# joshspeagle/dynesty

Measured on AMD Instinct MI355X. Metric: proposals/sec + ellipsoid-rebuilds/sec, 25-D corr-Normal nlive=2000 (multi/rwalk), higher is better.
Workload: dtype f64; 1 GPU; C2 x 64 independent runs per GPU (C5 shard); per step and run: 1 MultiEllipsoid rebuild + enlarge 1.25 + 4 queue fills of K=512 walkers x 45 rwalk steps (= one bound-update interval at the queue size that passes the ln Z gate); live sets uniform inside the likelihood contour; ndim=25, nlive=2000, walks=45, queue_size=512, runs_per_gpu=64, tap_point=A (kernel boundary), rebuild_in_step=True, rng=PCG64 + ziggurat, stream-identical to numpy.random.Generator (parity mode)

## Files before the change

### dynesty_amd/csrc/rebuild.hip

```cpp
#include <math.h>
#include <stdlib.h>

#include "ctx.h"
#include <type_traits>
#include <vector>
#include "eig_wave.h"

using namespace dh;
using dh_eig::jacobi_wave;
using dh_eig::sort_eigs_wave;
using dh_eig::wave_sync;

namespace {

constexpr int kThreads = 256;
constexpr double kRoundDelta = 1e-3;
constexpr double kMaxCond = 1e12;
constexpr double kEigMult = 10.0;
constexpr int kNTries = 100;

struct Node {
  int start, count;
  int parent, child0, child1;
  int depth;
// ... 1202 lines not shown
    PH_ADD(15);
    return L.lam[0] > 0.0 && isfinite(L.lam[0]);
  }
  __shared__ double s_q;
  if (t < 64) {
    double y = 0.0;
    if (t < D)
      for (int k = 0; k < D; ++k) y = fma(L.AX[t * LD + k], s_v[k], y);
    const double q = wave_sum(t < D ? y * s_v[t] : 0.0);
    if (t == 0) s_q = q;
  }
  __syncthreads();
  {
    const double q = s_q, rq = sqrt(q);
    for (int e = t; e < D * D; e += NT) {
      const int i = e / D, jj = e - i * D, o = i * LD + jj;
      Q[o] = L.AX[o];
      L.AX[o] = jj == 0 ? s_v[i] * rq : 0.0;
    }
    if (t < D) L.lam[t] = t == 0 ? q : 0.0;
    if (cov_keep) *cov_keep = Q;
    __syncthreads();
    PH_ADD(15);
    return q > 0.0 && isfinite(q);
  }
}

template <int NT = kThreads>
__device__ __forceinline__ int ellipsoid_finish_fast(const Lds& L, const RebuildArgs& a, double* es, double* cov_g,
                                                     const double* cov_keep, double fmx, double logdet,
                                                     double* logvol_out) {
  const int D = a.d, t = threadIdx.x, LD = L.LD, DD = D * D;
  if (!isfinite(logdet)) return DH_ERR_VALUE;
  const double lim = 1.0 - kRoundDelta;
  const bool sc = fmx > lim;
  const double mult = fmx / lim, rt = sqrt(mult);
  if (t < D) {
    st_c(L, es + t, L.mean[t]);
    double lam = L.lam[t];
    if (sc) lam *= mult;
    st_c(L, es + D + 3 * DD + t, sqrt(lam));
  }
  for (int e = t; e < DD; e += NT) {
    const int i = e / D, j = e - i * D, o = i * LD + j;
    double c = cov_keep[o], am = L.AM[o], ax = L.AX[o];
    if (sc) {
      c *= mult;
      am /= mult;
      ax *= rt;
      cov_g[o] = c;
    }
    st_c(L, es + D + e, c);
    st_c(L, es + D + DD + e, am);
    st_c(L, es + D + 2 * DD + e, ax);
  }
  *logvol_out = a.prefactor + 0.5 * logdet;
  return DH_OK;
}

template <int NT = kThreads>
__device__ __forceinline__ void ellipsoid_rescale(const Lds& L, double* cov_g, int D, double fmx) {
  const int t = threadIdx.x, LD = L.LD;
  const double lim = 1.0 - kRoundDelta;
  if (fmx > lim) {
    const double mult = fmx / lim;
    const double rt = sqrt(mult);
    for (int e = t; e < D * D; e += NT) {
      const int i = e / D, j = e % D;
      cov_g[i * LD + j] *= mult;
      L.AM[i * LD + j] /= mult;
      L.AX[i * LD + j] *= rt;
    }
    __syncthreads();
    if (t < D) L.lam[t] *= mult;
    __syncthreads();
  }
}

__device__ __forceinline__ int ellipsoid_store(const Lds& L, const RebuildArgs& a, double* es, const double* cov_g,
                                               double* logvol_out) {
  const int D = a.d, t = threadIdx.x, LD = L.LD;
  bool ok = true;
  double slog = 0.0;
  for (int k = 0; k < D; ++k) {
    const double l = L.lam[k];
    if (!(l > 0.0) || !isfinite(l)) ok = false;
    slog += log(l);
  }
  if (!ok) return DH_ERR_VALUE;
  const double logvol = a.prefactor + 0.5 * slog;
  const int DD = D * D;
  if (t < D) {
    st_c(L, es + t, L.mean[t]);
    st_c(L, es + D + 3 * DD + t, sqrt(L.lam[t]));
  }
  for (int e = t; e < DD; e += kThreads) {
    const int i = e / D, j = e % D;
    st_c(L, es + D + e, cov_g[i * LD + j]);
    st_c(L, es + D + DD + e, L.AM[i * LD + j]);
    st_c(L, es + D + 2 * DD + e, L.AX[i * LD + j]);
  }
  __syncthreads();
  *logvol_out = logvol;
  return DH_OK;
}

template <int NT = kThreads>
__device__ __forceinline__ int ellipsoid_store_fast(const Lds& L, const RebuildArgs& a, double* es,
                                                    const double* cov_g, double logdet, double* logvol_out) {
  const int D = a.d, t = threadIdx.x, LD = L.LD;
  if (!isfinite(logdet)) return DH_ERR_VALUE;
  const int DD = D * D;
  if (t < D) {
    st_c(L, es + t, L.mean[t]);
    st_c(L, es + D + 3 * DD + t, sqrt(L.lam[t]));
  }
  for (int e = t; e < DD; e += NT) {
    const int i = e / D, j = e % D;
    st_c(L, es + D + e, cov_g[i * LD + j]);
    st_c(L, es + D + DD + e, L.AM[i * LD + j]);
    st_c(L, es + D + 2 * DD + e, L.AX[i * LD + j]);
  }
  __syncthreads();
  *logvol_out = a.prefactor + 0.5 * logdet;
  return DH_OK;
}

constexpr int kFullRecord = 1;

constexpr int kDeferred = 3;
template <bool FAST, bool CHILD = false>
__device__ __forceinline__ int node_ellipsoid(const Lds& L, const RebuildArgs& a, const double* pts, const int* perm,
                                              int start, int count, double* es, double* cov_g, double* logvol_out,
                                              double* fmax_out, bool have_mean = false) {
  const int D = a.d, t = threadIdx.x, LD = L.LD;
  if (count == 1) return DH_ERR_VALUE;
  PH_T0();
  if (CHILD || have_mean) {
    if (t < D) L.mean[t] = ld_c(L, es + t);
    __syncthreads();
  } else {
    node_mean(L, pts, perm, start, count, D);
  }
  PH_ADD(0);
  int fused = 0;
  node_cov(L, pts, perm, start, count, D, CHILD ? false : !have_mean, FAST ? cov_g : nullptr, &fused);
  PH_ADD(1);
  if (!fused) {
    for (int e = t; e < D * D; e += kThreads) cov_g[(e / D) * LD + e % D] = L.A[(e / D) * LD + e % D];
    __syncthreads();
  }
  if constexpr (FAST) {
    double logdet = 0.0;
    const double* cov_keep = nullptr;
    if (fused != 2 && spd_fast(L, cov_g, D, a.mode == 0 && count >= 4 * D, &logdet, &cov_keep, fused == 1)) {
      const double fmx = node_fmax(L, pts, perm, start, count, D);
      PH_ADD(3);
      if (fmx > 1.0 - kRoundDelta) logdet += (double)D * log(fmx / (1.0 - kRoundDelta));
      *fmax_out = fmin(fmx, 1.0 - kRoundDelta);
      if (cov_keep != nullptr) return ellipsoid_finish_fast(L, a, es, cov_g, cov_keep, fmx, logdet, logvol_out);
      ellipsoid_rescale(L, cov_g, D, fmx);
      return ellipsoid_store_fast(L, a, es, cov_g, logdet, logvol_out);
    }
    if constexpr (CHILD) return kDeferred;
    __syncthreads();
    for (int pass = 0; pass < 2; ++pass) {
      const bool good = regularize<false>(L, cov_g, D);
      const double fmx = node_fmax(L, pts, perm, start, count, D);
      if (pass == 0) ellipsoid_rescale(L, cov_g, D, fmx);
      if (pass == 1 && fmx >= 1.0) return DH_ERR_CONTAIN;
      *fmax_out = pass == 0 ? fmin(fmx, 1.0 - kRoundDelta) : fmx;
      if (good) break;
    }
    const int rc = ellipsoid_store(L, a, es, cov_g, logvol_out);
    return rc == DH_OK ? kFullRecord : rc;
  } else {
    for (int pass = 0; pass < 2; ++pass) {
      const bool good = regularize(L, cov_g, D);
      PH_ADD(2);
      const double fmx = node_fmax(L, pts, perm, start, count, D);
      PH_ADD(3);
      if (pass == 0) ellipsoid_rescale(L, cov_g, D, fmx);
      if (pass == 1 && fmx >= 1.0) return DH_ERR_CONTAIN;
      *fmax_out = pass == 0 ? fmin(fmx, 1.0 - kRoundDelta) : fmx;
      if (good) break;
    }
    return ellipsoid_store(L, a, es, cov_g, logvol_out);
  }
}


constexpr int kBarSleep = 4;
__device__ __forceinline__ void drain_stores() {
  __builtin_amdgcn_s_waitcnt(0x0F70);
}

typedef double dh_d2 __attribute__((ext_vector_type(2)));
__device__ __forceinline__ void st_agent16(double* p, double v, unsigned long long tag) {
  dh_d2 x;
  x.x = v;
  x.y = __longlong_as_double((long long)tag);
  asm volatile("global_store_dwordx4 %0, %1, off sc1\n\ts_nop 1" ::"v"(p), "v"(x) : "memory");
}
__device__ __forceinline__ void ld_agent16x8(const double* const (&p)[8], dh_d2 (&v)[8]) {
  asm volatile(
      "global_load_dwordx4 %0, %8, off sc1\n\t"
      "global_load_dwordx4 %1, %9, off sc1\n\t"
      "global_load_dwordx4 %2, %10, off sc1\n\t"
      "global_load_dwordx4 %3, %11, off sc1\n\t"
      "global_load_dwordx4 %4, %12, off sc1\n\t"
      "global_load_dwordx4 %5, %13, off sc1\n\t"
      "global_load_dwordx4 %6, %14, off sc1\n\t"
      "global_load_dwordx4 %7, %15, off sc1\n\t"
      "s_waitcnt vmcnt(0)"
      : "=&v"(v[0]), "=&v"(v[1]), "=&v"(v[2]), "=&v"(v[3]), "=&v"(v[4]), "=&v"(v[5]), "=&v"(v[6]), "=&v"(v[7])
      : "v"(p[0]), "v"(p[1]), "v"(p[2]), "v"(p[3]), "v"(p[4]), "v"(p[5]), "v"(p[6]), "v"(p[7])
      : "memory");
}

template <bool MAXOP = false>
__device__ __forceinline__ double tagged_partner_reduce(const double* base, size_t stride, int col, int np,
                                                        unsigned long long tag, bool* ok) {
  double acc = MAXOP ? -INFINITY : 0.0;
  for (int pp0 = 0; pp0 < np && *ok; pp0 += 8) {
    const double* ptr[8];
    dh_d2 v[8];
#pragma unroll
    for (int uu = 0; uu < 8; ++uu) ptr[uu] = base + ((size_t)min(pp0 + uu, np - 1) * stride + col) * 2;
    for (int spins = 0;; ++spins) {
      ld_agent16x8(ptr, v);
      bool all = true;
#pragma unroll
      for (int uu = 0; uu < 8; ++uu) all = all && (unsigned long long)__double_as_longlong(v[uu].y) == tag;
      if (all) break;
      if (spins > (1 << 18)) {
        *ok = false;
        break;
      }
      __builtin_amdgcn_s_sleep(1);
    }
#pragma unroll
    for (int uu = 0; uu < 8; ++uu) {
      if (MAXOP)
        acc = pp0 + uu < np ? fmax(acc, v[uu].x) : acc;
      else
        acc += pp0 + uu < np ? v[uu].x : 0.0;
    }
  }
  return acc;
}

__device__ __forceinline__ bool parts_barrier(int* bar, int target) {
  __shared__ int ok_flag;
  drain_stores();
  __syncthreads();
  if (threadIdx.x == 0) {
    __hip_atomic_fetch_add(bar, 1, __ATOMIC_RELAXED, __HIP_MEMORY_SCOPE_AGENT);
    int ok = 1;
    long long spins = 0;
    while (__hip_atomic_load(bar, __ATOMIC_RELAXED, __HIP_MEMORY_SCOPE_AGENT) < target) {
      __builtin_amdgcn_s_sleep(kBarSleep);
      if (++spins > (1ll << 20)) {
        ok = 0;
        break;
      }
    }
    ok_flag = ok;
  }
  __syncthreads();
  return ok_flag != 0;
}

template <bool NB3>
__device__ __forceinline__ void kmeans_label_sums(const Lds& L, unsigned long long sel, double& o0, double& o1, double& o2) {
  const int lane = threadIdx.x & 63, w = threadIdx.x >> 6, LD = L.LD;
  const int lj = lane & 15, lk = lane >> 4;
  double a0 = 0.0, a1 = 0.0, a2 = 0.0, b0 = 0.0, b1 = 0.0, b2 = 0.0;
  const unsigned long long mine = sel >> lk;
  const double* base = L.tile + (w * 64 + lk) * LD + lj;
#pragma unroll 1
  for (int h = 0; h < 2; ++h) {
#pragma unroll
    for (int g = 0; g < 4; ++g) {
      const int g8 = h * 4 + g;
      const double ind = ((mine >> (8 * g8)) & 1ull) ? 1.0 : 0.0;
      const double indb = ((mine >> (8 * g8 + 4)) & 1ull) ? 1.0 : 0.0;
      const double* row = base + g8 * 8 * LD;
      const double* rowb = row + 4 * LD;
      a0 = DH_MFMA_F64_4X4(ind, row[0], a0);
      b0 = DH_MFMA_F64_4X4(indb, rowb[0], b0);
      a1 = DH_MFMA_F64_4X4(ind, row[16], a1);
      b1 = DH_MFMA_F64_4X4(indb, rowb[16], b1);
      if constexpr (NB3) {
        a2 = DH_MFMA_F64_4X4(ind, row[32], a2);
        b2 = DH_MFMA_F64_4X4(indb, rowb[32], b2);
      }
    }
  }
  o0 = a0 + b0;
  o1 = a1 + b1;
  o2 = a2 + b2;
}

__device__ __forceinline__ double readlane_f64(double v, int l) {
  const long long b = __double_as_longlong(v);
  const unsigned lo = (unsigned)__builtin_amdgcn_readlane((int)(unsigned)b, l);
  const unsigned hi = (unsigned)__builtin_amdgcn_readlane((int)(unsigned)((unsigned long long)b >> 32), l);
  return __longlong_as_double((long long)(((unsigned long long)hi << 32) | lo));
}

constexpr int kLloydIters = 10;
static_assert(kLloydIters + 1 <= 0xff, "the iteration tag has 8 bits");

__device__ int node_kmeans_part(const Lds& L, const double* pts, int* perm, int* perm2, int start, int count,
                                int D, const double* es, int q, int np, double* kp0, double* kp1, int* bar,
                                int min_size, unsigned long long tag0, int lvl = 0) {
  LV_T0();
  const int t = threadIdx.x, lane = t & 63, w = t >> 6, LD = L.LD;
  const int DD = D * D, KP = 2 * D + 2;
  const int s0 = start + q * L.TP, cnt = min(L.TP, count - q * L.TP);
  if (t < D) L.sums[t] = ld_c(L, es + D + 3 * DD + t);
  __syncthreads();
  if (t == 0) {
    L.ri[303] = 0;
    int best = 0;
    double bl = L.sums[0];
    for (int k = 1; k < D; ++k)
      if (L.sums[k] > bl) {
        bl = L.sums[k];
        best = k;
      }
    L.ri[301] = best;
  }
  stage_tile(L, pts, perm, s0, cnt, D, 0);
  const int kbest = L.ri[301];
  if (t < D) {
    const double v = ld_c(L, es + D + 2 * DD + t * D + kbest), ct = ld_c(L, es + t);
    L.cen[t] = (ct - v) / L.scale[t];
    L.cen[D + t] = (ct + v) / L.scale[t];
  }
  __syncthreads();
  const int nb = (D + 15) >> 4;
  const int lj = lane & 15, lk = lane >> 4;
  int lb = 0, lb_prev = -1, n0 = 0, c0_tile = 0, last_it = kLloydIters - 1;
  LV_ADD(lvl, 0);
  LV_SET(lvl, 5, np);
  LV_SET(lvl, 6, count);
  PH_T0();
  {
    const int rup = min(L.TP, (cnt + 63) & ~63);
    const int jz = t & (L.DP - 1), pz0 = cnt + (t >> L.DPlog), pzs = kThreads >> L.DPlog;
    if (jz < D)
      for (int pz = pz0; pz < rup; pz += pzs) L.tile[pz * LD + jz] = 0.0;
    __syncthreads();
  }
  unsigned long long m0 = 0ull, m1 = 0ull;
  for (int it = 0; it < kLloydIters; ++it) {
    const bool has = t < cnt;
    if (w * 64 < cnt) {
      const double c0l = L.cen[lane < D ? lane : 0], c1l = L.cen[D + (lane < D ? lane : 0)];
      const double* x = L.tile + (has ? t : 0) * LD;
      double d0 = 0.0, d1 = 0.0;
      for (int j0 = 0; j0 < D; j0 += 8) {
        double xv[8];
#pragma unroll
        for (int u = 0; u < 8; ++u) xv[u] = x[min(j0 + u, D - 1)];
#pragma unroll
        for (int u = 0; u < 8; ++u)
          if (j0 + u < D) {
            const double e0 = xv[u] - readlane_f64(c0l, j0 + u), e1 = xv[u] - readlane_f64(c1l, j0 + u);
            d0 = fma(e0, e0, d0);
            d1 = fma(e1, e1, d1);
          }
      }
      lb = d1 < d0 ? 1 : 0;
    }
    LV_ADD(lvl, 8);
    {
      const unsigned long long mv = __ballot(has && lb != lb_prev);
      m1 = __ballot(has && lb == 1);
      m0 = __ballot(has && lb == 0);
      if (lane == 0) {
        L.ri[260 + w] = __popcll(mv);
        L.ri[264 + w] = __popcll(m0);
      }
      lb_prev = lb;
    }
    __syncthreads();
    c0_tile = L.ri[264] + L.ri[265] + L.ri[266] + L.ri[267];
    const int ch_tile = L.ri[260] + L.ri[261] + L.ri[262] + L.ri[263];
    PH_ADD(10);
    LV_ADD(lvl, 9);
    double a0 = 0.0, a1 = 0.0, a2 = 0.0;
    if (w * 64 < cnt) {
      const int li = lane & 3;
      const unsigned long long sel = li == 0 ? m0 : li == 1 ? m1 : 0ull;
      if (nb > 2)
        kmeans_label_sums<true>(L, sel, a0, a1, a2);
      else
        kmeans_label_sums<false>(L, sel, a0, a1, a2);
    }
    if (lane < 32) {
      double* o = L.kred + (w * 2 + lk) * 48;
      o[lj] = a0;
      if (nb > 1) o[16 + lj] = a1;
      if (nb > 2) o[32 + lj] = a2;
    }
    LV_ADD(lvl, 10);
    __syncthreads();
    PH_ADD(11);
    LV_ADD(lvl, 11);
    double* kp = (it & 1) ? kp1 : kp0;
    if (t < 2 * D) {
      const int c = t >= D ? 1 : 0, j = t - c * D;
      double sum = 0.0;
      for (int g0 = 0; g0 < kThreads / 64; g0 += L.KG) {
        double gs = 0.0;
        for (int wv = g0; wv < g0 + L.KG; ++wv) gs += L.kred[(wv * 2 + c) * 48 + j];
        sum += gs;
      }
      L.sums[c * D + j] = sum;
      if (np == 1) {
        const int nc = c ? count - c0_tile : c0_tile;
        if (nc > 0) L.cen[c * D + j] = sum / (double)nc;
      }
    }
    n0 = c0_tile;
    LV_ADD(lvl, 12);
    if (np > 1) {
      const unsigned long long tag = tag0 + (unsigned long long)(it + 1);
      if (t < KP) {
        const double mine = t < 2 * D ? L.sums[t] : t == 2 * D ? (double)c0_tile : (double)ch_tile;
        st_agent16(kp + ((size_t)q * KP + t) * 2, mine, tag);
        double sum = 0.0;
        bool ok = true;
        for (int pp0 = 0; pp0 < np && ok; pp0 += 8) {
          const double* ptr[8];
          dh_d2 v[8];
#pragma unroll
          for (int uu = 0; uu < 8; ++uu) ptr[uu] = kp + ((size_t)min(pp0 + uu, np - 1) * KP + t) * 2;
          for (int spins = 0;; ++spins) {
            ld_agent16x8(ptr, v);
            bool all = true;
#pragma unroll
            for (int uu = 0; uu < 8; ++uu) all = all && (unsigned long long)__double_as_longlong(v[uu].y) == tag;
            if (all) break;
            if (spins > (1 << 18)) {
              ok = false;
              break;
            }
            __builtin_amdgcn_s_sleep(1);
          }
#pragma unroll
          for (int uu = 0; uu < 8; ++uu) sum += pp0 + uu < np ? v[uu].x : 0.0;
        }
        if (!ok) L.ri[303] = 1;
        L.sums[t] = sum;
      }
      __syncthreads();
      if (L.ri[303]) return -1;
      n0 = (int)L.sums[2 * D];
    }
    LV_ADD(lvl, 13);
    const int moved = np > 1 ? (int)L.sums[2 * D + 1] : ch_tile;
    if (np > 1) {
      const int n1 = count - n0;
      if (t < D) {
        if (n0 > 0) L.cen[t] = L.sums[t] / (double)n0;
        if (n1 > 0) L.cen[D + t] = L.sums[D + t] / (double)n1;
      }
    }
    __syncthreads();
    PH_ADD(12);
    LV_ADD(lvl, 14);
    if (moved == 0) {
      last_it = it;
      break;
    }
  }
  LV_ADD(lvl, 1);
  LV_SET(lvl, 4, last_it + 1);
  if (min(n0, count - n0) < min_size) return n0;
  const bool valid = t < cnt;
  const unsigned long long pm0 = __ballot(valid && lb == 0);
  const unsigned long long lt = (1ull << lane) - 1ull;
  if (lane == 0) L.ri[256 + w] = __popcll(pm0);
  __syncthreads();
  int before0 = 0;
  for (int wv = 0; wv < w; ++wv) before0 += L.ri[256 + wv];
  const int rank0 = before0 + __popcll(pm0 & lt);
  int off0 = 0, off1 = n0;
  if (np > 1) {
    const double* kp = (last_it & 1) ? kp1 : kp0;
    for (int pp0 = 0; pp0 < q; pp0 += 8) {
      double part[8];
#pragma unroll
      for (int uu = 0; uu < 8; ++uu)
      {
        const double pv8 = ld_agent(kp + ((size_t)min(pp0 + uu, q - 1) * KP + 2 * D) * 2);
        part[uu] = pp0 + uu < q ? pv8 : 0.0;
      }
#pragma unroll
      for (int uu = 0; uu < 8; ++uu)
        if (pp0 + uu < q) {
          off0 += (int)part[uu];
          off1 += L.TP - (int)part[uu];
        }
    }
  }
  if (valid) {
    const int pos = lb == 0 ? off0 + rank0 : off1 + (t - rank0);
    const int src = ld_ci(L, perm + s0 + t);
    if (np > 1 || L.coh)
      st_agent_i(perm2 + start + pos, src);
    else
      perm2[start + pos] = src;
  }
  if (np > 1) {
    if (!parts_barrier(bar, np)) return -1;
    if (valid) st_ci(L, perm + s0 + t, ld_agent_i(perm2 + s0 + t));
  } else if (L.coh) {
    drain_stores();
    __syncthreads();
    if (valid) st_agent_i(perm + s0 + t, ld_agent_i(perm2 + s0 + t));
  } else {
    __threadfence_block();
    __syncthreads();
    if (valid) perm[s0 + t] = perm2[s0 + t];
  }
  LV_ADD(lvl, 2);
  return n0;
}

__device__ __forceinline__ double logaddexp_d(double x, double y) {
  if (x == y) return x + 0.6931471805599453;
  const double d = x - y;
  if (d > 0) return x + log1p(exp(-d));
  if (d <= 0) return y + log1p(exp(d));
  return x + y;
}


constexpr size_t kLdsLimit = 159 * 1024;
constexpr size_t kLdsSeparate = 79 * 1024;
__host__ __device__ inline size_t rebuild_lds_base_bytes(int D, int TP) {
  const int LD = D | 1;
  const size_t dbl = (size_t)TP * LD + 4 * (size_t)D * LD + 7 * (size_t)D + 2 + kThreads + 128;
  return (dbl * 8 + (320 + (size_t)D + 8) * 4 + 15) & ~(size_t)15;
}

__device__ __forceinline__ void carve(Lds& L, unsigned char* smem, int D, int TP = kThreads) {
  L.LD = D | 1;
  L.TP = TP;
  L.c_pts = nullptr;
  L.c_start = L.c_cnt = L.c_how = -1;
  L.coh = false;
  L.KG = kThreads / 64;
  L.DP = 1;
  L.DPlog = 0;
  while (L.DP < D) {
    L.DP <<= 1;
    ++L.DPlog;
  }
  double* p = (double*)smem;
  L.tile = p;
  p += (size_t)L.TP * L.LD;
  L.A = p;
  p += D * L.LD;
  L.V = p;
  p += D * L.LD;
  L.AM = p;
  p += D * L.LD;
  L.AX = p;
  p += D * L.LD;
  L.mean = p;
  p += D;
  L.scale = p;
  p += D;
  L.lam = p;
  p += D;
  L.cen = p;
  p += 2 * D;
  L.sums = p;
  p += 2 * D + 2;
  L.red = p;
  p += kThreads;
  L.rc = p;
  p += 64;
  L.rs = p;
  p += 64;
  L.kred = L.red;
  L.ibuf = (int*)L.red;
  L.ibuf_cap = 2 * (kThreads + 128);
  L.ri = (int*)p;
  L.perm_sort = L.ri + 320;
  const int P = (D + 1) & ~1;
  L.JLD = P | 1;
  const size_t jdbl = 4 * (size_t)P * L.JLD;
  L.j_alias = rebuild_lds_base_bytes(D, TP) + jdbl * 8 > kLdsSeparate;
  double* jb = L.j_alias ? L.tile : (double*)(smem + rebuild_lds_base_bytes(D, TP));
  L.JA[0] = jb;
  L.JA[1] = jb + (size_t)P * L.JLD;
  L.JV[0] = jb + 2 * (size_t)P * L.JLD;
  L.JV[1] = jb + 3 * (size_t)P * L.JLD;
}

__host__ __device__ inline size_t split_lds_bytes(int D, int TP) {
  const int LD = D | 1;
  return ((((size_t)TP * LD + 5 * (size_t)D + 2 + kThreads + 128) * 8 + (320 + (size_t)D + 8) * 4) + 15) & ~(size_t)15;
}

__device__ __forceinline__ void carve_split(Lds& L, unsigned char* smem, int D, int TP) {
  L.LD = D | 1;
  L.TP = TP;
  L.c_pts = nullptr;
  L.c_start = L.c_cnt = L.c_how = -1;
  L.coh = false;
  L.KG = kThreads / 64;
  L.DP = 1;
  L.DPlog = 0;
  while (L.DP < D) {
    L.DP <<= 1;
    ++L.DPlog;
  }
  double* p = (double*)smem;
  L.tile = p;
  p += (size_t)TP * L.LD;
  L.scale = p;
  p += D;
  L.cen = p;
  p += 2 * D;
  L.sums = p;
  p += 2 * D + 2;
  L.red = p;
  L.rc = p + kThreads;
  L.rs = L.rc + 64;
  L.kred = L.red;
  L.ibuf = (int*)L.red;
  L.ibuf_cap = 2 * (kThreads + 128);
  p += kThreads + 128;
  L.ri = (int*)p;
  L.perm_sort = L.ri + 320;
  L.A = L.V = L.AM = L.AX = L.mean = L.lam = nullptr;
  L.JA[0] = L.JA[1] = L.JV[0] = L.JV[1] = nullptr;
  L.JLD = 0;
  L.j_alias = false;
}

struct RunView {
  const double* pts;
  int* perm;
  int* perm2;
  unsigned char* lab;
  Node* nodes;
  double* estore;
  int* reslist;
  int NS, ES;
};

__device__ __forceinline__ RunView view_of(const RebuildArgs& a, int run, int LD) {
  RunView v;
  const int D = a.d;
  v.pts = a.pts + (size_t)run * a.n * D;
  v.perm = a.perm + (size_t)run * a.n;
  v.perm2 = a.perm2 + (size_t)run * a.n;
  v.lab = a.lab + (size_t)run * a.n;
  v.nodes = a.nodes + (size_t)run * a.max_nodes;
  v.ES = D + 3 * D * D + D;
  v.NS = v.ES + D * LD;
  v.estore = a.estore + (size_t)run * a.max_nodes * v.NS;
  v.reslist = a.reslist + (size_t)run * a.reslist_cap;
  return v;
}

__device__ __forceinline__ void set_status(const RebuildArgs& a, int run, int rc) {
  if (threadIdx.x == 0 && rc != DH_OK) atomicMin(&a.status[run], rc);
}

constexpr unsigned long long kItemValid = 1ull << 63, kItemSplit = 1ull << 62;
__device__ __forceinline__ unsigned long long tq_item(bool split, int run, int node, int part) {
  return kItemValid | (split ? kItemSplit : 0ull) | ((unsigned long long)run << 40) | ((unsigned long long)node << 16) |
         (unsigned long long)part;
}
__device__ __forceinline__ bool tq_push(const RebuildArgs& a, bool split, int run, int node0, int n) {
  __hip_atomic_fetch_add(a.tq_ctl + 32, n, __ATOMIC_RELAXED, __HIP_MEMORY_SCOPE_AGENT);
  const int s0 = __hip_atomic_fetch_add(a.tq_ctl + 16, n, __ATOMIC_RELAXED, __HIP_MEMORY_SCOPE_AGENT);
  if (s0 + n > a.tq_cap) {
    __hip_atomic_fetch_add(a.tq_ctl + 32, -n, __ATOMIC_RELAXED, __HIP_MEMORY_SCOPE_AGENT);
    atomicMin(&a.status[run], DH_ERR_NOMEM);
    return false;
  }
  for (int i = 0; i < n; ++i)
    __hip_atomic_store(a.tq_items + s0 + i, split ? tq_item(true, run, node0, i) : tq_item(false, run, node0 + i, 0),
                       __ATOMIC_RELAXED, __HIP_MEMORY_SCOPE_AGENT);
  return true;
}

__device__ __forceinline__ void queue_split(const RebuildArgs& a, int run, int level, int node, int count) {
  if (a.tree || level >= a.tree_from) {
    const int np = (count + a.tps - 1) / a.tps;
    int* nb = a.nbar + ((size_t)run * a.max_nodes + node) * kBarStride;
    int pb = 0;
    if (np > 1) {
      pb = atomicAdd(&a.kp_top[run], np);
      if (pb + np > a.kp_cap) {
        atomicMin(&a.status[run], DH_ERR_NOMEM);
        return;
      }
    }
    st_agent_i(nb + 2, pb);
    __builtin_amdgcn_s_waitcnt(0x0F70);
    (void)tq_push(a, true, run, node, np);
    return;
  }
  const size_t lp = (size_t)(level & 1) * a.runs + run;
  const int sidx = atomicAdd(&a.nsplit[(size_t)level * a.runs + run], 1);
  const int np = (count + a.tps - 1) / a.tps;
  const int pb = atomicAdd(&a.nparts[(size_t)level * a.runs + run], np);
  if (sidx >= a.maxw || pb + np > a.maxp) {
    atomicMin(&a.status[run], DH_ERR_NOMEM);
    return;
  }
  a.split_list[lp * a.maxw + sidx] = node;
  a.part_base[lp * a.maxw + sidx] = pb;
  for (int qq = 0; qq < np; ++qq) {
    a.part_list[(lp * a.maxp + pb + qq) * 2] = sidx;
    a.part_list[(lp * a.maxp + pb + qq) * 2 + 1] = qq;
  }
}

__global__ void __launch_bounds__(kThreads, 2) k_root_parts(RebuildArgs a, int rp) {
  extern __shared__ __attribute__((aligned(16))) unsigned char smem[];
  PH_LEVEL(-1);
  const int D = a.d, DD = D * D, t = threadIdx.x, run = a.root_run0 + blockIdx.x / rp, q = blockIdx.x % rp;
  const int n = a.n_arr ? a.n_arr[run] : a.n;
  if (a.active && !a.active[run]) return;
  Lds L;
  carve(L, smem, D);
  const int np = (n > 1 && rp > 1) ? (n + L.TP - 1) / L.TP : 1;
  if (q >= np) return;
  const RunView v = view_of(a, run, L.LD);
  const int LD = L.LD;
  const int s0 = q * L.TP, cnt = min(L.TP, n - s0);
  for (int p = s0 + t; p < (np == 1 ? n : s0 + cnt); p += kThreads) v.perm[p] = p;
  __threadfence_block();
  __syncthreads();
  double* es = v.estore;
  double* cov_g = v.estore + v.ES;
  int status = DH_OK;
  double lv = 0.0;
  int root_fast = 0;
  double root_logdet = 0.0;
  double root_fmax = INFINITY;
  if (np == 1) {
    if (n <= 1) status = (a.mode == 0) ? DH_ERR_REGION : DH_ERR_VALUE;
    if (status == DH_OK) {
      if (a.fast) {
        status = node_ellipsoid<true>(L, a, v.pts, v.perm, 0, n, es, cov_g, &lv, &root_fmax);
        root_fast = status == DH_OK;
        if (status == kFullRecord) status = DH_OK;
      } else {
        status = node_ellipsoid<false>(L, a, v.pts, v.perm, 0, n, es, cov_g, &lv, &root_fmax);
      }
    }
  } else {
    double* rb = a.rootbuf + (size_t)run * a.rootbuf_stride;
    double* b_sum = rb;
    double* b_sq = b_sum + (size_t)rp * D * 2;
    double* b_cov = b_sq + (size_t)rp * D * 2;
    double* b_am = b_cov + (size_t)rp * DD * 2;
    double* b_fmx = b_am + (size_t)DD * 2;
    double* b_flag = b_fmx + (size_t)rp * 2;
    const unsigned long long tg = ((unsigned long long)a.epoch << 8) | 0x8000000000000000ull;
    __shared__ int s_bad;
    if (t == 0) s_bad = 0;
    const int G = kThreads / D > 0 ? kThreads / D : 1;
    const int j = t % D, g = t / D;
    const bool want_split = a.mode == 0 && n >= 4 * D;
    bool ok = true;
    stage_tile(L, v.pts, v.perm, s0, cnt, D, 0);
    {
      double acc = 0.0;
      if (t < G * D)
        for (int p = g; p < cnt; p += G) acc += L.tile[p * LD + j];
      L.red[t] = acc;
      __syncthreads();
      if (t < D) {
        double sum = 0.0;
        for (int gg = 0; gg < G; ++gg) sum += L.red[gg * D + t];
        st_agent16(b_sum + ((size_t)q * D + t) * 2, sum, tg + 1);
        L.mean[t] = tagged_partner_reduce(b_sum, D, t, np, tg + 1, &ok) / (double)n;
      }
    }
    __syncthreads();
    stage_tile(L, v.pts, v.perm, s0, cnt, D, 1);
    {
      mfma_acc acc[6];
#pragma unroll
      for (int b = 0; b < 6; ++b) acc[b] = (mfma_acc){0.0, 0.0, 0.0, 0.0};
      tile_cov_accumulate(L, cnt, D, acc);
      __syncthreads();
      cov_fold_waves(L, D, acc);
      for (int e = t; e < DD; e += kThreads) {
        const int i = e / D, k = e - i * D;
        if (i <= k) st_agent16(b_cov + ((size_t)q * DD + e) * 2, L.A[i * LD + k], tg + 2);
      }
    }
    if (want_split) {
      double acc = 0.0;
      if (t < G * D)
        for (int p = g; p < cnt; p += G) {
          const double x = L.tile[p * LD + j];
          acc = fma(x, x, acc);
        }
      __syncthreads();
      L.red[t] = acc;
      __syncthreads();
      if (t < D) {
        double sum = 0.0;
        for (int gg = 0; gg < G; ++gg) sum += L.red[gg * D + t];
        st_agent16(b_sq + ((size_t)q * D + t) * 2, sum, tg + 2);
      }
    }
    int flag = 0;
    if (q == 0) {
      for (int e = t; e < DD; e += kThreads) {
        const int i = e / D, k = e - i * D;
        if (i <= k) L.A[i * LD + k] = tagged_partner_reduce(b_cov, DD, e, np, tg + 2, &ok);
      }
      if (!ok) s_bad = 1;
      __syncthreads();
      cov_finalize(L, D, 1.0 / (double)(n - 1));
      for (int e = t; e < DD; e += kThreads) cov_g[(e / D) * LD + e % D] = L.A[(e / D) * LD + e % D];
      __syncthreads();
      if (a.fast && spd_fast(L, cov_g, D, want_split, &root_logdet)) root_fast = 1;
      const bool good = root_fast || regularize(L, cov_g, D);
      flag = good ? 1 : 2;
      if (good)
        for (int e = t; e < DD; e += kThreads) st_agent16(b_am + (size_t)e * 2, L.AM[(e / D) * LD + e % D], tg + 3);
      if (t == 0) st_agent16(b_flag, (double)flag, tg + 3);
    }
    if (want_split) {
      if (t < D) L.scale[t] = sqrt(tagged_partner_reduce(b_sq, D, t, np, tg + 2, &ok) / (double)n);
      if (!ok) s_bad = 1;
      __syncthreads();
      double* ps = a.pts_scaled + (size_t)run * a.n * D;
      const int jj = t & (L.DP - 1), p0 = t >> L.DPlog, pstep = kThreads >> L.DPlog;
      if (jj < D) {
        const double sj = L.scale[jj];
        for (int p = s0 + p0; p < s0 + cnt; p += pstep) ps[(size_t)p * D + jj] = v.pts[(size_t)p * D + jj] / sj;
      }
      if (q == 0 && t < D) a.scale_g[(size_t)run * D + t] = L.scale[t];
    }
    if (q > 0) {
      if (t == 0) {
        bool ok1 = true;
        flag = (int)tagged_partner_reduce(b_flag, 1, 0, 1, tg + 3, &ok1);
        if (!ok1) s_bad = 1;
        L.ri[300] = flag;
      }
      __syncthreads();
      flag = L.ri[300];
    }
    if (flag == 1) {
      if (q > 0) {
        for (int e = t; e < DD; e += kThreads) L.AM[(e / D) * LD + e % D] = tagged_partner_reduce(b_am, 1, e, 1, tg + 3, &ok);
        if (!ok) s_bad = 1;
        __syncthreads();
      }
      stage_tile(L, v.pts, v.perm, s0, cnt, D, 1);
      double best = -INFINITY;
      if (D >= kMfmaMinDim) {
        best = tile_quadform_max(L, L.AM, cnt, D, best);
      } else {
        for (int p = t; p < cnt; p += kThreads) {
          const double* x = L.tile + p * LD;
          double qf = 0.0;
          for (int i = 0; i < D; ++i) {
            double r = 0.0;
            const double* row = L.AM + i * LD;
            for (int k = 0; k < D; ++k) r = fma(row[k], x[k], r);
            qf = fma(x[i], r, qf);
          }
          best = fmax(best, qf);
        }
      }
      __syncthreads();
      best = block_reduce_max(best, L.red);
      if (t == 0) st_agent16(b_fmx + (size_t)q * 2, best, tg + 4);
      if (q == 0) {
        if (t == 0) {
          bool ok1 = true;
          L.red[0] = tagged_partner_reduce<true>(b_fmx, 1, 0, np, tg + 4, &ok1);
          if (!ok1) s_bad = 1;
        }
        __syncthreads();
        const double fmx = L.red[0];
        __syncthreads();
        if (s_bad) status = DH_ERR_HIP;
        if (root_fast && fmx > 1.0 - kRoundDelta) root_logdet += (double)D * log(fmx / (1.0 - kRoundDelta));
        ellipsoid_rescale(L, cov_g, D, fmx);
        root_fmax = fmin(fmx, 1.0 - kRoundDelta);
        if (status == DH_OK)
          status = root_fast ? ellipsoid_store_fast(L, a, es, cov_g, root_logdet, &lv)
                             : ellipsoid_store(L, a, es, cov_g, &lv);
      }
    } else if (q == 0) {
      __syncthreads();
      if (s_bad) status = DH_ERR_HIP;
      if (status == DH_OK) {
        for (int p = t; p < n; p += kThreads) v.perm[p] = p;
        __threadfence_block();
        __syncthreads();
        status = node_ellipsoid<false>(L, a, v.pts, v.perm, 0, n, es, cov_g, &lv, &root_fmax);
      }
    }
    __syncthreads();
    if (q > 0) {
      if (s_bad && t == 0) atomicMin(&a.kerr[run], DH_ERR_HIP);
    } else {
      if (s_bad) status = DH_ERR_HIP;
      if (t == 0 && status == DH_OK && want_split) queue_split(a, run, 0, 0, n);
    }
  }
  if (q == 0 && t == 0) {
    Node r;
    r.start = 0;
    r.count = n;
    r.parent = -1;
    r.child0 = r.child1 = -1;
    r.depth = 0;
    r.split = 0;
    r.res_start = 0;
    r.res_len = 0;
    r.fast = root_fast;
    r.has_mean = 0;
    r.logvol = lv;
    r.fmax = root_fmax;
    v.nodes[0] = r;
    a.nnodes_dev[run] = 1;
    a.status[run] = status;
  }
  if (np == 1 && status == DH_OK && a.mode == 0 && n >= 4 * D) {
    {
      const Lds Lc = L;
      node_std(Lc, v.pts, v.perm, 0, n, D);
      L.c_pts = nullptr;
    }
    if (t < D) a.scale_g[(size_t)run * D + t] = L.scale[t];
    double* ps = a.pts_scaled + (size_t)run * a.n * D;
    const int jj = t & (L.DP - 1), p0 = t >> L.DPlog, pstep = kThreads >> L.DPlog;
    if (jj < D) {
      const double sj = L.scale[jj];
      for (int p = p0; p < n; p += pstep) ps[(size_t)p * D + jj] = v.pts[(size_t)p * D + jj] / sj;
    }
    if (t == 0) queue_split(a, run, 0, 0, n);
  }
}

__device__ __forceinline__ void split_body(const RebuildArgs& a, const Lds& L, const RunView& v, int run, int level, int slot, int q,
                           bool single) {
  const int D = a.d, t = threadIdx.x;
  const size_t lp = (size_t)(level & 1) * a.runs + run;
  const bool tq = a.tree == 1;
  int* nb = tq ? a.nbar + ((size_t)run * a.max_nodes + slot) * kBarStride : nullptr;
  const int pb = tq ? ld_agent_i(nb + 2) : a.part_base[lp * a.maxw + slot];
  const int cur = a.tree ? slot : a.split_list[lp * a.maxw + slot];
  const int start = ld_ci(L, &v.nodes[cur].start), count = ld_ci(L, &v.nodes[cur].count),
            depth = ld_ci(L, &v.nodes[cur].depth);
  const int np = single ? 1 : (count + L.TP - 1) / L.TP;
  const int min_size = 2 * D;
  const int KP = 2 * D + 2;
  double* kp0 = a.kpart + ((size_t)run * a.maxp + pb) * KP * 2;
  double* kp1 = kp0 + (size_t)a.runs * a.maxp * KP * 2;
  const unsigned long long tag0 = ((unsigned long long)a.epoch << 24) | ((unsigned long long)(level & 0xffff) << 8);
  int* bar = a.tree ? nb : a.kbar + (((size_t)level * a.runs + run) * a.maxw + slot) * kBarStride;
  PH_T0();
  const int n0 = node_kmeans_part(L, a.pts_scaled + (size_t)run * a.n * D, v.perm, v.perm2, start, count, D,
                                  v.estore + (size_t)cur * v.NS, q, np, kp0, kp1, bar, min_size, tag0, level);
  PH_ADD(4);
  LV_T0();
  if (n0 < 0) {
    if (t == 0) atomicMin(a.tree ? &a.status[run] : &a.kerr[run], DH_ERR_HIP);
    return;
  }
  const int n1 = count - n0;
  if (min(n0, n1) < min_size) return;
  bool creator = q == 0;
  if (tq) {
    drain_stores();
    __syncthreads();
    if (t == 0)
      L.ri[302] = __hip_atomic_fetch_add(nb + 1, 1, __ATOMIC_RELAXED, __HIP_MEMORY_SCOPE_AGENT) == np - 1 ? 1 : 0;
    __syncthreads();
    creator = L.ri[302] != 0;
  }
  if (creator && t == 0) {
    L.ri[300] = -1;
    const int c0 = atomicAdd(&a.nnodes_dev[run], 2);
    if (c0 + 2 > a.max_nodes) {
      atomicMin(a.tree ? &a.status[run] : &a.kerr[run], DH_ERR_NOMEM);
    } else {
      Node k0, k1;
      k0.start = start;
      k0.count = n0;
      k1.start = start + n0;
      k1.count = n1;
      k0.parent = k1.parent = cur;
      k0.child0 = k0.child1 = k1.child0 = k1.child1 = -1;
      k0.depth = k1.depth = depth + 1;
      k0.split = k1.split = 0;
      k0.res_start = k1.res_start = 0;
      k0.res_len = k1.res_len = 0;
      k0.fast = k1.fast = 0;
      k0.has_mean = k1.has_mean = 1;
      k0.logvol = k1.logvol = 0.0;
      k0.fmax = k1.fmax = INFINITY;
      if (a.tree) {
        static_assert(sizeof(Node) % 4 == 0, "Node is copied as ints");
        const int* w0 = (const int*)&k0;
        const int* w1 = (const int*)&k1;
        int* d0 = (int*)&v.nodes[c0];
        int* d1 = (int*)&v.nodes[c0 + 1];
        for (int i = 0; i < (int)(sizeof(Node) / 4); ++i) {
          st_agent_i(d0 + i, w0[i]);
          st_agent_i(d1 + i, w1[i]);
        }
        st_agent_i(&v.nodes[cur].child0, c0);
        st_agent_i(&v.nodes[cur].child1, c0 + 1);
        st_agent_i(&v.nodes[cur].split, 1);
      } else {
        v.nodes[c0] = k0;
        v.nodes[c0 + 1] = k1;
        v.nodes[cur].child0 = c0;
        v.nodes[cur].child1 = c0 + 1;
        v.nodes[cur].split = 1;
        const int e = atomicAdd(&a.nell[(size_t)level * a.runs + run], 2);
        int* el = a.ell_list + ((size_t)level * a.runs + run) * 2 * a.maxw;
        el[e] = c0;
        el[e + 1] = c0 + 1;
      }
      L.ri[300] = c0;
    }
  }
  if (creator) {
    if (t == 0 && !(L.ri[300] >= 0 && L.ri[300] + 2 <= a.max_nodes)) L.ri[300] = -1;
    __syncthreads();
    const int c0 = L.ri[300];
    if (c0 >= 0 && t < 2 * D) {
      const int c = t >= D ? 1 : 0, j = t - c * D;
      st_c(L, v.estore + (size_t)(c0 + c) * v.NS + j, L.cen[c * D + j] * L.scale[j]);
    }
    if (a.tree && c0 >= 0) {
      drain_stores();
      __syncthreads();
      if (tq && t == 0) (void)tq_push(a, false, run, c0, 2);
    }
  }
  LV_ADD(level, 3);
}

__device__ __forceinline__ void k_split_impl(const RebuildArgs& a, int level, int gp, int cr);
#ifndef DH_KSPLIT_WAVES
#define DH_KSPLIT_WAVES 5
#endif
__global__ void __launch_bounds__(kThreads, DH_KSPLIT_WAVES) k_split(RebuildArgs a, int level, int gp, int cr) {
  WG_STAMP(0, level, 0);
  PH_LEVEL(-1);
  k_split_impl(a, level, gp, cr);
  WG_STAMP(0, level, 1);
}
__device__ __forceinline__ void k_split_impl(const RebuildArgs& a, int level, int gp, int cr) {
  extern __shared__ __attribute__((aligned(16))) unsigned char smem[];
  const int per = cr * gp, chunk = blockIdx.x / per, b = blockIdx.x - chunk * per;
  const int rc = min(cr, a.runs - chunk * cr);
  const int run = chunk * cr + b % rc, ps = b / rc;
  if (ps >= gp) return;
  const int nps = a.nparts[(size_t)level * a.runs + run];
  if (nps > gp) {
    if (threadIdx.x == 0) atomicMin(&a.kerr[run], DH_ERR_NOMEM);
    return;
  }
  if (ps >= nps) return;
  if (a.status[run] != DH_OK) return;
  const int D = a.d, t = threadIdx.x;
  Lds L;
  carve_split(L, smem, D, a.tps);
  const RunView v = view_of(a, run, L.LD);
  if (t < D) L.scale[t] = a.scale_g[(size_t)run * D + t];
  __syncthreads();
  const size_t lp = (size_t)(level & 1) * a.runs + run;
  const int slot = a.part_list[(lp * a.maxp + ps) * 2], q = a.part_list[(lp * a.maxp + ps) * 2 + 1];
  split_body(a, L, v, run, level, slot, q, false);
}

template <bool SLOW, bool DEFER = false>
__device__ __forceinline__ bool ell_body(const RebuildArgs& a, const Lds& L, const RunView& v, int run, int level, int node) {
  const int D = a.d, t = threadIdx.x;
  const int start = ld_ci(L, &v.nodes[node].start), count = ld_ci(L, &v.nodes[node].count);
  double lv = 0.0, fmx = INFINITY;
  __syncthreads();
  L.c_pts = nullptr;
  int rc;
  if constexpr (DEFER) {
    rc = v.nodes[node].has_mean ? node_ellipsoid<true, true>(L, a, v.pts, v.perm, start, count, v.estore + (size_t)node * v.NS,
                                                             v.estore + (size_t)node * v.NS + v.ES, &lv, &fmx, true)
                                : kDeferred;
    if (rc == kDeferred) {
      if (t == 0) (void)tq_push(a, false, run, node, 1);
      return true;
    }
  } else {
    rc = node_ellipsoid<!SLOW>(L, a, v.pts, v.perm, start, count, v.estore + (size_t)node * v.NS,
                               v.estore + (size_t)node * v.NS + v.ES, &lv, &fmx,
                               ld_ci(L, &v.nodes[node].has_mean) != 0);
  }
  const bool full = SLOW || rc == kFullRecord;
  if (rc != DH_OK && rc != kFullRecord) {
    set_status(a, run, rc);
    return false;
  }
  if (a.tree) {
    drain_stores();
    __syncthreads();
  }
  if (t == 0) {
    v.nodes[node].logvol = lv;
    v.nodes[node].fmax = fmx;
    v.nodes[node].fast = full ? 0 : 1;
    if (count >= 4 * D) {
      if (!a.tree && a.tree_from > a.levels && level + 1 >= a.levels) {
        atomicMin(&a.status[run], DH_ERR_NOMEM);
      } else {
        queue_split(a, run, level + 1, node, count);
      }
    }
  }
  return true;
}

template <bool SLOW, bool DEFER>
__device__ __forceinline__ void k_ell_impl(const RebuildArgs& a, int level, int G, int skip_done, int tp);
template <bool SLOW, bool DEFER = false>
__global__ void __launch_bounds__(kThreads, SLOW ? 1 : 2) k_ell(RebuildArgs a, int level, int G, int skip_done, int tp) {
  WG_STAMP(1, level, 0);
  PH_LEVEL(level);
  k_ell_impl<SLOW, DEFER>(a, level, G, skip_done, tp);
  WG_STAMP(1, level, 1);
}
template <bool SLOW, bool DEFER>
__device__ __forceinline__ void k_ell_impl(const RebuildArgs& a, int level, int G, int skip_done, int tp) {
  extern __shared__ __attribute__((aligned(16))) unsigned char smem[];
  const int run = blockIdx.x % a.runs, g = blockIdx.x / a.runs;
  const int* list = a.ell_list + ((size_t)level * a.runs + run) * 2 * a.maxw;
  const int cnt = a.nell[(size_t)level * a.runs + run];
  if (g >= cnt) return;
  if (a.kerr[run] != DH_OK) {
    if (threadIdx.x == 0) atomicMin(&a.status[run], a.kerr[run]);
    return;
  }
  if (a.status[run] != DH_OK) return;
  const int D = a.d;
  Lds L;
  carve(L, smem, D, tp);
  const RunView v = view_of(a, run, L.LD);
  for (int slot = g; slot < cnt; slot += G) {
    if (skip_done && v.nodes[list[slot]].fmax < INFINITY) continue;
    if (!ell_body<SLOW, DEFER>(a, L, v, run, level, list[slot])) return;
  }
}

constexpr int kWaveDeclined = 2;
constexpr int kWaveCap = 128;

__host__ __device__ inline size_t wave_lds_bytes(int D) {
  const int LD = D | 1;
  return ((((size_t)kWaveCap * LD + 4 * (size_t)D * LD + 2 * (size_t)D + 64) * 8) + 15) & ~(size_t)15;
}

__device__ __forceinline__ void carve_wave(Lds& L, unsigned char* smem, int D) {
  L.LD = D | 1;
  L.TP = kWaveCap;
  L.c_pts = nullptr;
  L.c_start = L.c_cnt = L.c_how = -1;
  L.coh = false;
  L.KG = 1;
  L.DP = 1;
  L.DPlog = 0;
  while (L.DP < D) {
    L.DP <<= 1;
    ++L.DPlog;
  }
  double* p = (double*)smem;
  L.tile = p;
  p += (size_t)kWaveCap * L.LD;
  L.A = p;
  p += D * L.LD;
  L.AM = p;
  p += D * L.LD;
  L.V = p;
  p += D * L.LD;
  L.AX = p;
  p += D * L.LD;
  L.mean = p;
  p += D;
  L.lam = p;
  p += D;
  L.red = p;
  L.ibuf = (int*)L.red;
  L.ibuf_cap = 128;
  L.scale = L.cen = L.sums = L.rc = L.rs = L.kred = nullptr;
  L.ri = L.perm_sort = nullptr;
  L.JA[0] = L.JA[1] = L.JV[0] = L.JV[1] = nullptr;
  L.JLD = 0;
  L.j_alias = false;
}

__device__ __forceinline__ int node_ellipsoid_wave(const Lds& L, const RebuildArgs& a, const double* pts, const int* perm,
                                                   int start, int count, double* es, double* cov_g,
                                                   double* logvol_out, double* fmax_out) {
  const int D = a.d, t = threadIdx.x, LD = L.LD;
  if (t < D) L.mean[t] = es[t];
  __syncthreads();
  stage_tile<64>(L, pts, perm, start, count, D, 1);
  {
    const int nb = (D + 15) >> 4, lane = t & 63, lj = lane & 15, lk = lane >> 4;
    for (int wv = 0; wv * 64 < count; ++wv) {
      mfma_acc acc[6];
#pragma unroll
      for (int b = 0; b < 6; ++b) acc[b] = (mfma_acc){0.0, 0.0, 0.0, 0.0};
      tile_cov_accumulate(L, count, D, acc, wv);
#pragma unroll
      for (int b = 0; b < 6; ++b) {
        const int ib = b == 0 ? 0 : b == 1 ? 0 : b == 2 ? 1 : b == 3 ? 0 : b == 4 ? 1 : 2;
        const int jb = b == 0 ? 0 : b == 1 ? 1 : b == 2 ? 1 : 2;
        if (jb < nb) {
#pragma unroll
          for (int r = 0; r < 4; ++r) {
            const int i = ib * 16 + lk + 4 * r, j = jb * 16 + lj;
            if (i < D && j < D) {
              double v = acc[b][r];
              if (wv > 0) v += L.A[i * LD + j];
              L.A[i * LD + j] = v;
            }
          }
        }
      }
      __syncthreads();
    }
  }
  cov_finalize<64>(L, D, 1.0 / (double)(count - 1));
  for (int e = t; e < D * D; e += 64) cov_g[(e / D) * LD + e % D] = L.A[(e / D) * LD + e % D];
  __syncthreads();
  double logdet = 0.0;
  if (!spd_fast<64>(L, cov_g, D, a.mode == 0 && count >= 4 * D, &logdet)) return kWaveDeclined;
  const double fmx = node_fmax<64>(L, pts, perm, start, count, D);
  if (fmx > 1.0 - kRoundDelta) logdet += (double)D * log(fmx / (1.0 - kRoundDelta));
  ellipsoid_rescale<64>(L, cov_g, D, fmx);
  *fmax_out = fmin(fmx, 1.0 - kRoundDelta);
  return ellipsoid_store_fast<64>(L, a, es, cov_g, logdet, logvol_out);
}

__global__ void __launch_bounds__(64, 3) k_ell_wave(RebuildArgs a, int level, int G) {
  extern __shared__ __attribute__((aligned(16))) unsigned char smem[];
  PH_LEVEL(-1);
  const int run = blockIdx.x % a.runs, g = blockIdx.x / a.runs;
  const int* list = a.ell_list + ((size_t)level * a.runs + run) * 2 * a.maxw;
  const int cnt = a.nell[(size_t)level * a.runs + run];
  if (g >= cnt) return;
  if (a.kerr[run] != DH_OK || a.status[run] != DH_OK) return;
  const int D = a.d, t = threadIdx.x;
  Lds L;
  carve_wave(L, smem, D);
  const RunView v = view_of(a, run, L.LD);
  for (int slot = g; slot < cnt; slot += G) {
    const int node = list[slot];
    const int start = v.nodes[node].start, count = v.nodes[node].count;
    if (!v.nodes[node].has_mean || count < 2 || count > kWaveCap) continue;
    double lv = 0.0, fmx = INFINITY;
    __syncthreads();
    L.c_pts = nullptr;
    const int rc = node_ellipsoid_wave(L, a, v.pts, v.perm, start, count, v.estore + (size_t)node * v.NS,
// ... 1176 lines not shown
```

Measured before the change: 2.896 billion proposals/s.

## Add wide k-means path splitting centroid distances across half-waves with DPP broadcasts

Adds a templated wide variant of the k-means partition for 128-point tiles and dimensions 8 to 48. In it, each half-wave computes the distance to one of the two centroids, using DPP row broadcasts and compile-time-unrolled chains instead of per-coordinate readlane. The two halves then compare their distances with a lane xor. Label masks are shared through LDS as 32-bit words, and the MFMA label-sum loop uses a single accumulator chain. This is meant to cut the serial readlane cost of the Lloyd assignment step, at the price of more template instantiations, larger code size and extra LDS mask traffic.

```diff
diff --git a/dynesty_amd/csrc/rebuild.hip b/dynesty_amd/csrc/rebuild.hip
--- a/dynesty_amd/csrc/rebuild.hip
+++ b/dynesty_amd/csrc/rebuild.hip
@@ -1528,6 +1528,72 @@
   o2 = a2 + b2;
 }
 
+template <bool NB3>
+__device__ __forceinline__ void kmeans_label_sums_chain(const Lds& L, unsigned long long sel, double& o0, double& o1, double& o2) {
+  const int lane = threadIdx.x & 63, w = threadIdx.x >> 6, LD = L.LD;
+  const int lj = lane & 15, lk = lane >> 4, cb = (w >> 1) * 4;
+  double a0 = 0.0, a1 = 0.0, a2 = 0.0;
+  const unsigned long long mine = sel >> (lk + cb);
+  const double* base = L.tile + ((w & 1) * 64 + cb + lk) * LD + lj;
+#pragma unroll 4
+  for (int g8 = 0; g8 < 8; ++g8) {
+    const double ind = ((mine >> (8 * g8)) & 1ull) ? 1.0 : 0.0;
+    const double* row = base + g8 * 8 * LD;
+    a0 = DH_MFMA_F64_4X4(ind, row[0], a0);
+    a1 = DH_MFMA_F64_4X4(ind, row[16], a1);
+    if constexpr (NB3) a2 = DH_MFMA_F64_4X4(ind, row[32], a2);
+  }
+  o0 = a0;
+  o1 = a1;
+  o2 = a2;
+}
+
+template <int I>
+__device__ __forceinline__ double row_bcast_f64(double v) {
+  static_assert(I >= 0 && I < 16, "a lane of the row");
+  return __builtin_amdgcn_mov_dpp(v, 0x150 + I, 0xF, 0xF, false);
+}
+template <int J>
+__device__ __forceinline__ double sqdist_step(double d, double x, double c0, double c1, double c2) {
+  const double e = x - row_bcast_f64<(J & 15)>(J < 16 ? c0 : J < 32 ? c1 : c2);
+  return fma(e, e, d);
+}
+template <int J0, int ND>
+__device__ __forceinline__ double sqdist_blocks(const double* x, double d, const double (&xv)[8], double c0, double c1, double c2) {
+  constexpr int N = ND - J0 < 8 ? ND - J0 : 8, NN = ND - J0 - 8 < 8 ? ND - J0 - 8 : 8;
+  double xn[8] = {0.0, 0.0, 0.0, 0.0, 0.0, 0.0, 0.0, 0.0};
+  if constexpr (NN > 0) {
+#pragma unroll
+    for (int u = 0; u < NN; ++u) xn[u] = x[J0 + 8 + u];
+  }
+  if constexpr (N > 0) d = sqdist_step<J0 + 0>(d, xv[0], c0, c1, c2);
+  if constexpr (N > 1) d = sqdist_step<J0 + 1>(d, xv[1], c0, c1, c2);
+  if constexpr (N > 2) d = sqdist_step<J0 + 2>(d, xv[2], c0, c1, c2);
+  if constexpr (N > 3) d = sqdist_step<J0 + 3>(d, xv[3], c0, c1, c2);
+  if constexpr (N > 4) d = sqdist_step<J0 + 4>(d, xv[4], c0, c1, c2);
+  if constexpr (N > 5) d = sqdist_step<J0 + 5>(d, xv[5], c0, c1, c2);
+  if constexpr (N > 6) d = sqdist_step<J0 + 6>(d, xv[6], c0, c1, c2);
+  if constexpr (N > 7) d = sqdist_step<J0 + 7>(d, xv[7], c0, c1, c2);
+  if constexpr (NN > 0)
+    return sqdist_blocks<J0 + 8, ND>(x, d, xn, c0, c1, c2);
+  else
+    return d;
+}
+template <int ND>
+__device__ __forceinline__ double sqdist_chain(const double* x, double c0, double c1, double c2) {
+  static_assert(ND >= 1 && ND <= 48, "three registers of sixteen coordinates");
+  double xv[8] = {0.0, 0.0, 0.0, 0.0, 0.0, 0.0, 0.0, 0.0};
+#pragma unroll
+  for (int u = 0; u < (ND < 8 ? ND : 8); ++u) xv[u] = x[u];
+  double d = sqdist_blocks<0, ND>(x, 0.0, xv, c0, c1, c2);
+  asm volatile("" : "+v"(d));
+  return d;
+}
+#define DH_WIDE_DIMS(X)                                                                                               \
+  X(8) X(9) X(10) X(11) X(12) X(13) X(14) X(15) X(16) X(17) X(18) X(19) X(20) X(21) X(22) X(23) X(24) X(25) X(26) X(27) \
+  X(28) X(29) X(30) X(31) X(32) X(33) X(34) X(35) X(36) X(37) X(38) X(39) X(40) X(41) X(42) X(43) X(44) X(45) X(46)   \
+  X(47) X(48)
+
 __device__ __forceinline__ double readlane_f64(double v, int l) {
   const long long b = __double_as_longlong(v);
   const unsigned lo = (unsigned)__builtin_amdgcn_readlane((int)(unsigned)b, l);
@@ -1535,9 +1601,12 @@
   return __longlong_as_double((long long)(((unsigned long long)hi << 32) | lo));
 }
 
+__device__ __forceinline__ bool kmeans_wide_form(const Lds& L, int D) { return L.TP == 128 && D >= 8 && D <= 48; }
+
 constexpr int kLloydIters = 10;
 static_assert(kLloydIters + 1 <= 0xff, "the iteration tag has 8 bits");
 
+template <bool WIDE>
 __device__ int node_kmeans_part(const Lds& L, const double* pts, int* perm, int* perm2, int start, int count,
                                 int D, const double* es, int q, int np, double* kp0, double* kp1, int* bar,
                                 int min_size, unsigned long long tag0, int lvl = 0) {
@@ -1581,9 +1650,31 @@
     __syncthreads();
   }
   unsigned long long m0 = 0ull, m1 = 0ull;
+  constexpr bool wide = WIDE;
+  const int half = lane >> 5, pw = (w << 5) | (lane & 31);
+  const int wu = __builtin_amdgcn_readfirstlane(w);
+  const int cg = cnt - (wu & 1) * 64;
   for (int it = 0; it < kLloydIters; ++it) {
-    const bool has = t < cnt;
-    if (w * 64 < cnt) {
+    const bool has = wide ? pw < cnt : t < cnt;
+    if (wide) {
+      if (w * 32 < cnt) {
+        const double* cn = L.cen + half * D + (lane & 15);
+        const double c0r = cn[0], c1r = cn[16], c2r = cn[32];
+        const double* x = L.tile + (has ? pw : 0) * LD;
+        double d = 0.0;
+        switch (D) {
+#define DH_SQD_CASE(N) \
+  case N:              \
+    d = sqdist_chain<N>(x, c0r, c1r, c2r); \
+    break;
+          DH_WIDE_DIMS(DH_SQD_CASE)
+#undef DH_SQD_CASE
+          default: break;
+        }
+        const double dp = xor_lane<32>(d);
+        lb = (half ? d < dp : dp < d) ? 1 : 0;
+      }
+    } else if (w * 64 < cnt) {
       const double c0l = L.cen[lane < D ? lane : 0], c1l = L.cen[D + (lane < D ? lane : 0)];
       const double* x = L.tile + (has ? t : 0) * LD;
       double d0 = 0.0, d1 = 0.0;
@@ -1605,20 +1696,43 @@
     {
       const unsigned long long mv = __ballot(has && lb != lb_prev);
       m1 = __ballot(has && lb == 1);
-      m0 = __ballot(has && lb == 0);
-      if (lane == 0) {
-        L.ri[260 + w] = __popcll(mv);
-        L.ri[264 + w] = __popcll(m0);
+      if (wide) {
+        const int nv = __popc((unsigned)__ballot(has));
+        if (lane == 0) {
+          L.ri[260 + w] = __popc((unsigned)mv);
+          L.ri[264 + w] = nv - __popc((unsigned)m1);
+          L.ri[268 + w] = (int)(unsigned)m1;
+        }
+      } else {
+        m0 = __ballot(has && lb == 0);
+        if (lane == 0) {
+          L.ri[260 + w] = __popcll(mv);
+          L.ri[264 + w] = __popcll(m0);
+        }
       }
       lb_prev = lb;
     }
     __syncthreads();
     c0_tile = L.ri[264] + L.ri[265] + L.ri[266] + L.ri[267];
     const int ch_tile = L.ri[260] + L.ri[261] + L.ri[262] + L.ri[263];
+    if (wide) {
+      const int g2 = (wu & 1) * 2;
+      m1 = (unsigned long long)(unsigned)L.ri[268 + g2] | ((unsigned long long)(unsigned)L.ri[269 + g2] << 32);
+      m0 = ~m1 & (cg >= 64 ? ~0ull : cg > 0 ? (1ull << cg) - 1ull : 0ull);
+    }
     PH_ADD(10);
     LV_ADD(lvl, 9);
     double a0 = 0.0, a1 = 0.0, a2 = 0.0;
-    if (w * 64 < cnt) {
+    if (wide) {
+      if (cg > 0) {
+        const int li = lane & 3;
+        const unsigned long long sel = li == 0 ? m0 : li == 1 ? m1 : 0ull;
+        if (nb > 2)
+          kmeans_label_sums_chain<true>(L, sel, a0, a1, a2);
+        else
+          kmeans_label_sums_chain<false>(L, sel, a0, a1, a2);
+      }
+    } else if (w * 64 < cnt) {
       const int li = lane & 3;
       const unsigned long long sel = li == 0 ? m0 : li == 1 ? m1 : 0ull;
       if (nb > 2)
@@ -1640,10 +1754,17 @@
     if (t < 2 * D) {
       const int c = t >= D ? 1 : 0, j = t - c * D;
       double sum = 0.0;
-      for (int g0 = 0; g0 < kThreads / 64; g0 += L.KG) {
+      if (wide) {
         double gs = 0.0;
-        for (int wv = g0; wv < g0 + L.KG; ++wv) gs += L.kred[(wv * 2 + c) * 48 + j];
+        gs += L.kred[(0 * 2 + c) * 48 + j] + L.kred[(2 * 2 + c) * 48 + j];
+        gs += L.kred[(1 * 2 + c) * 48 + j] + L.kred[(3 * 2 + c) * 48 + j];
         sum += gs;
+      } else {
+        for (int g0 = 0; g0 < kThreads / 64; g0 += L.KG) {
+          double gs = 0.0;
+          for (int wv = g0; wv < g0 + L.KG; ++wv) gs += L.kred[(wv * 2 + c) * 48 + j];
+          sum += gs;
+        }
       }
       L.sums[c * D + j] = sum;
       if (np == 1) {
@@ -1707,6 +1828,7 @@
   LV_ADD(lvl, 1);
   LV_SET(lvl, 4, last_it + 1);
   if (min(n0, count - n0) < min_size) return n0;
+  if (wide) lb = (L.ri[268 + (t >> 5)] >> (t & 31)) & 1;
   const bool valid = t < cnt;
   const unsigned long long pm0 = __ballot(valid && lb == 0);
   const unsigned long long lt = (1ull << lane) - 1ull;
@@ -2202,8 +2324,11 @@
   const unsigned long long tag0 = ((unsigned long long)a.epoch << 24) | ((unsigned long long)(level & 0xffff) << 8);
   int* bar = a.tree ? nb : a.kbar + (((size_t)level * a.runs + run) * a.maxw + slot) * kBarStride;
   PH_T0();
-  const int n0 = node_kmeans_part(L, a.pts_scaled + (size_t)run * a.n * D, v.perm, v.perm2, start, count, D,
-                                  v.estore + (size_t)cur * v.NS, q, np, kp0, kp1, bar, min_size, tag0, level);
+  const double* kpts = a.pts_scaled + (size_t)run * a.n * D;
+  const double* kes = v.estore + (size_t)cur * v.NS;
+  const int n0 = kmeans_wide_form(L, D)
+                     ? node_kmeans_part<true>(L, kpts, v.perm, v.perm2, start, count, D, kes, q, np, kp0, kp1, bar, min_size, tag0, level)
+                     : node_kmeans_part<false>(L, kpts, v.perm, v.perm2, start, count, D, kes, q, np, kp0, kp1, bar, min_size, tag0, level);
   PH_ADD(4);
   LV_T0();
   if (n0 < 0) {
```

Result: faster. 3.040 billion proposals/s (median of 6 runs) (+5.0%).
